# rafaelvp-db/databricks-distributed-deep-learning

Measured on AMD Instinct MI355X. Metric: ResNet-50 images/sec (whole node), higher is better.
Workload: dtype bf16

## Files before the change

### csrc/kernels/skinny_gemm.hip

```cpp
#include "ddl_lds.h"

#include <algorithm>
#include <cstdlib>

namespace {

constexpr int TM = 64, NT = 256, NW = NT / 64;
enum Epi { EPI_PLAIN = 0, EPI_RES = 1, EPI_BNB = 2, EPI_RESBNB = 3 };
template <int EPI>
constexpr bool is_bnb() { return EPI == EPI_BNB || EPI == EPI_RESBNB; }
template <int N>
constexpr int mask_stride() { return TM * N / 8 > 1024 ? TM * N / 8 : 1024; }

struct SkParams {
    const bf16_t* A;
    const bf16_t* B;
    bf16_t* C;
    long M;
    int tiles, chunk;
    float* colstats;
    const bf16_t* res;
    const bf16_t* aux;
    const uint8_t* mask;
    const float* mean;
    const float* istd;
    uint32_t c_bytes;
};

template <int N, int K, int EPI>
__global__ __launch_bounds__(NT) void skinny_gemm_k(SkParams p) {
    constexpr int NCF = N / 64;
    constexpr int KK = K / 32;
    constexpr int ABYTES = TM * K * 2, BBYTES = N * K * 2, CBYTES = TM * N * 2;
    constexpr int OFF_A = BBYTES, OFF_C = OFF_A + 2 * ABYTES;
    constexpr int NCIMG = EPI == EPI_PLAIN ? 1 : 2;
    constexpr int OFF_M = OFF_C + NCIMG * CBYTES;
    constexpr int MS = mask_stride<N>();
    constexpr int LDS = OFF_M + (is_bnb<EPI>() ? 2 * MS : 0);
    __shared__ __attribute__((aligned(16))) char smem[LDS];
    const int tid = threadIdx.x, lane = tid & 63, wv = __builtin_amdgcn_readfirstlane(tid >> 6);
    const int g = lane >> 4, r16 = lane & 15;
    const int cb = wv * 16 * NCF;
    const uint32_t lds0 = (uint32_t)(uintptr_t)smem;
    const __amdgpu_buffer_rsrc_t crs = rsrc(p.C, p.c_bytes);
    const bf16_t* eop = (EPI == EPI_RES || EPI == EPI_RESBNB) ? p.res : p.aux;

    const int t0 = blockIdx.x * p.chunk, t1 = min(p.tiles, t0 + p.chunk);
    auto prefetch = [&](int t, int buf) {
        dma_rows<NW, K, TM>(p.A, (long)t * TM, p.M, smem + OFF_A + buf * ABYTES, wv, lane);
        if constexpr (EPI != EPI_PLAIN) dma_rows<NW, N, TM>(eop, (long)t * TM, p.M, smem + OFF_C + buf * CBYTES, wv, lane);
        if constexpr (is_bnb<EPI>()) {
            const long byte0 = (long)t * TM * (N / 8), last = p.M * (N / 8) - 4;
#pragma unroll
            for (int k = 0; k < TM * N / 8 / 256; ++k) {
                const long b = min(byte0 + (long)(k * 64 + lane) * 4, last);
                const uint8_t* src = p.mask ? p.mask + b : (const uint8_t*)p.A;
                glds4(src, smem + OFF_M + buf * MS + k * 256);
            }
        }
    };
    uint2 xa[4][NCF], xb[4][NCF];
    auto prefetch_x = [&](int t, uint2 (&dst)[4][NCF]) {
#pragma unroll
        for (int i = 0; i < 4; ++i) {
            const long row = min((long)t * TM + 16 * i + r16, p.M - 1);
#pragma unroll
            for (int j = 0; j < NCF; ++j)
                dst[i][j] = *reinterpret_cast<const uint2*>(p.aux + row * N + cb + 16 * j + 4 * g);
        }
    };
    dma_rows<NW, K, N>(p.B, 0, N, smem, wv, lane);
    if (t0 < t1) {
        prefetch(t0, 0);
        if constexpr (EPI == EPI_RESBNB) prefetch_x(t0, xa);
    }

    uint32_t aoff[4][KK], boff[NCF][KK];
#pragma unroll
    for (int kk = 0; kk < KK; ++kk) {
#pragma unroll
        for (int i = 0; i < 4; ++i) {
            const int r = 16 * i + r16;
            aoff[i][kk] = r * (K * 2) + (((kk * 4 + g) ^ (r & swm<K>())) << 4);
        }
#pragma unroll
        for (int j = 0; j < NCF; ++j) {
            const int r = cb + 16 * j + r16;
            boff[j][kk] = lds0 + r * (K * 2) + (((kk * 4 + g) ^ (r & swm<K>())) << 4);
        }
    }
    auto coff = [&](int i, int j) -> uint32_t {
        const int row = 16 * i + r16, c = (cb + 16 * j) / 8 + (g >> 1);
        return row * (N * 2) + ((c ^ (row & swm<N>())) << 4) + (g & 1) * 8;
    };

    float st_s[NCF][4], st_q[NCF][4];
#pragma unroll
    for (int j = 0; j < NCF; ++j)
#pragma unroll
        for (int e = 0; e < 4; ++e) st_s[j][e] = st_q[j][e] = 0.f;
    float bmu[NCF][4] = {}, bis[NCF][4] = {};
    if constexpr (is_bnb<EPI>()) {
#pragma unroll
        for (int j = 0; j < NCF; ++j) {
            load4(p.mean + cb + 16 * j + 4 * g, bmu[j]);
            load4(p.istd + cb + 16 * j + 4 * g, bis[j]);
        }
    }

    auto tile = [&](const int t, uint2 (&xc)[4][NCF], uint2 (&xn)[4][NCF]) __attribute__((always_inline)) {
        const int buf = (t - t0) & 1;
        if constexpr (EPI == EPI_RESBNB) {
            __builtin_amdgcn_s_waitcnt(0xF70 | (2 * NCF));
        } else {
            if (t == t0) asm volatile("s_waitcnt vmcnt(0)" ::: "memory");
            else asm volatile("s_waitcnt vmcnt(%0)" ::"n"(2 * NCF) : "memory");
        }
        __builtin_amdgcn_s_barrier();
        if (t + 1 < t1) prefetch(t + 1, buf ^ 1);
        if constexpr (EPI == EPI_RESBNB) prefetch_x(t + 1, xn);

        const uint32_t abase = lds0 + OFF_A + buf * ABYTES;
        f32x4 acc[4][NCF];
#pragma unroll
        for (int i = 0; i < 4; ++i)
#pragma unroll
            for (int j = 0; j < NCF; ++j) acc[i][j] = (f32x4){0.f, 0.f, 0.f, 0.f};
#pragma unroll
        for (int kk = 0; kk < KK; ++kk) {
            bf16x8 af[4], bfr[NCF];
#pragma unroll
            for (int i = 0; i < 4; ++i) af[i] = ds_read16(abase + aoff[i][kk]);
#pragma unroll
            for (int j = 0; j < NCF; ++j) bfr[j] = ds_read16(boff[j][kk]);
            asm volatile("s_waitcnt lgkmcnt(0)" ::: "memory");
            __builtin_amdgcn_sched_barrier(0);
#pragma unroll
            for (int i = 0; i < 4; ++i)
#pragma unroll
                for (int j = 0; j < NCF; ++j)
                    acc[i][j] = __builtin_amdgcn_mfma_f32_16x16x32_bf16(bfr[j], af[i], acc[i][j], 0, 0, 0);
            __builtin_amdgcn_sched_barrier(0);
        }

        const long m0 = (long)t * TM;
        const uint32_t cimg = lds0 + OFF_C + (EPI == EPI_PLAIN ? 0 : buf * CBYTES);
        uint32_t mwords[4][2] = {{~0u, ~0u}, {~0u, ~0u}, {~0u, ~0u}, {~0u, ~0u}};
        if constexpr (is_bnb<EPI>()) {
            if (p.mask) {
#pragma unroll
                for (int i = 0; i < 4; ++i) {
                    const uint32_t a = lds0 + OFF_M + buf * MS + (16 * i + r16) * (N / 8) + (cb & ~31) / 8;
                    if constexpr (NCF > 2) {
                        const uint2 w2 = ds_read8(a);
                        mwords[i][0] = w2.x;
                        mwords[i][1] = w2.y;
                    } else {
                        mwords[i][0] = ds_read32(a);
                    }
                }
            }
        }
        uint2 ev[4][NCF];
        if constexpr (EPI != EPI_PLAIN) {
#pragma unroll
            for (int i = 0; i < 4; ++i)
#pragma unroll
                for (int j = 0; j < NCF; ++j) ev[i][j] = ds_read8(cimg + coff(i, j));
        }
        asm volatile("s_waitcnt lgkmcnt(0)" ::: "memory");
        __builtin_amdgcn_sched_barrier(0);
#pragma unroll
        for (int i = 0; i < 4; ++i) {
            const bool ok = m0 + 16 * i + r16 < p.M;
#pragma unroll
            for (int j = 0; j < NCF; ++j) {
                float v[4] = {acc[i][j][0], acc[i][j][1], acc[i][j][2], acc[i][j][3]};
                float xv[4] = {0.f, 0.f, 0.f, 0.f};
                if constexpr (EPI != EPI_PLAIN) {
                    xv[0] = __uint_as_float(ev[i][j].x << 16);
                    xv[1] = __uint_as_float(ev[i][j].x & 0xffff0000u);
                    xv[2] = __uint_as_float(ev[i][j].y << 16);
                    xv[3] = __uint_as_float(ev[i][j].y & 0xffff0000u);
                }
                if constexpr (EPI == EPI_RES || EPI == EPI_RESBNB) {
#pragma unroll
                    for (int e = 0; e < 4; ++e) v[e] += xv[e];
                }
                if constexpr (EPI == EPI_RESBNB) {
                    xv[0] = __uint_as_float(xc[i][j].x << 16);
                    xv[1] = __uint_as_float(xc[i][j].x & 0xffff0000u);
                    xv[2] = __uint_as_float(xc[i][j].y << 16);
                    xv[3] = __uint_as_float(xc[i][j].y & 0xffff0000u);
                }
                if constexpr (is_bnb<EPI>()) {
                    const uint32_t bits = mwords[i][(((cb & 31) + 16 * j) >> 5)] >> (((cb + 16 * j) & 16) + 4 * g);
#pragma unroll
                    for (int e = 0; e < 4; ++e) v[e] = ((bits >> e) & 1u) ? v[e] : 0.f;
                }
                const uint32_t lo = pack2bf(v[0], v[1]), hi = pack2bf(v[2], v[3]);
                ds_write8(cimg + coff(i, j), make_uint2(lo, hi));
                if (EPI != EPI_RES && ok) {
                    const float tq[4] = {__uint_as_float(lo << 16), __uint_as_float(lo & 0xffff0000u),
                                         __uint_as_float(hi << 16), __uint_as_float(hi & 0xffff0000u)};
#pragma unroll
                    for (int e = 0; e < 4; ++e) {
                        st_s[j][e] += tq[e];
                        st_q[j][e] += is_bnb<EPI>() ? tq[e] * xv[e] : tq[e] * tq[e];
                    }
                }
            }
        }
        asm volatile("s_waitcnt lgkmcnt(0)" ::: "memory");
        __builtin_amdgcn_s_barrier();
        constexpr int RPI = 1024 / (N * 2), CPR = N * 2 / 16;
#pragma unroll
        for (int qq = 0; qq < 2 * NCF; ++qq) {
            const int q = qq * 4 + wv;
            const int row = q * RPI + lane / CPR, c = lane % CPR;
            const u32x4 d = __builtin_bit_cast(u32x4, ds_read16(cimg + row * (N * 2) + ((c ^ (row & swm<N>())) << 4)));
            asm volatile("s_waitcnt lgkmcnt(0)" ::: "memory");
            __builtin_amdgcn_sched_barrier(0);
            const long grow = m0 + row;
            const uint32_t off = grow < p.M ? (uint32_t)((grow * N + c * 8) * 2) : 0x80000000u;
            __builtin_amdgcn_raw_buffer_store_b128(d, crs, (int)off, 0, 0);
        }
    };
    if constexpr (EPI == EPI_RESBNB) {
        __builtin_amdgcn_s_waitcnt(0xF70);
        for (int t = t0; t < t1; t += 2) {
            tile(t, xa, xb);
            if (t + 1 < t1) tile(t + 1, xb, xa);
        }
    } else {
        for (int t = t0; t < t1; ++t) tile(t, xa, xb);
    }

    if (EPI != EPI_RES && p.colstats) {
        asm volatile("s_waitcnt vmcnt(0)" ::: "memory");
        __syncthreads();
        float* red = reinterpret_cast<float*>(smem);
        for (int t = tid; t < 2 * N; t += NT) red[t] = 0.f;
        __syncthreads();
#pragma unroll
        for (int j = 0; j < NCF; ++j)
#pragma unroll
            for (int e = 0; e < 4; ++e) {
                float a = row16_sum(st_s[j][e]), b = row16_sum(st_q[j][e]);
                if constexpr (is_bnb<EPI>()) b = (b - bmu[j][e] * a) * bis[j][e];
                if (r16 == 0) {
                    const int col = cb + 16 * j + 4 * g + e;
                    atomicAdd(&red[col], a);
                    atomicAdd(&red[N + col], b);
                }
            }
        __syncthreads();
        for (int t = tid; t < 2 * N; t += NT) p.colstats[(long)blockIdx.x * 2 * N + t] = red[t];
    }
}

template <int N, int K, int EPI>
int launch(const SkParams& p0, int grid, hipStream_t st) {
    SkParams p = p0;
    constexpr int lds = N * K * 2 + 2 * TM * K * 2 + (EPI == EPI_PLAIN ? 1 : 2) * TM * N * 2 +
                        (is_bnb<EPI>() ? 2 * mask_stride<N>() : 0);
    const int per_cu = std::max(1, std::min(4, (160 * 1024) / lds));
    int g = grid > 0 ? grid : 256 * per_cu;
    g = std::min(g, p.tiles);
    p.chunk = (p.tiles + g - 1) / g;
    g = (p.tiles + p.chunk - 1) / p.chunk;
    hipLaunchKernelGGL((skinny_gemm_k<N, K, EPI>), dim3(g), dim3(NT), 0, st, p);
    return g;
}

}

DDL_API int ddl_skinny_gemm(const void* A, const void* B, void* C, long M, int N, int K, float* colstats,
                            const void* res, const void* aux, const uint8_t* mask, const float* mean,
                            const float* istd, int grid, hipStream_t stream) {
    if (M < 1 || M * (long)N * 2 >= (1l << 31)) return -1;
    const bool n256 = N == 256 && K == 64, n64 = N == 64 && K == 256;
    if (!n256 && !n64) return -1;
    if (res && !n256) return -1;
    if (aux && (!mean || !istd || (n256 && !res))) return -1;
    SkParams p{};
    p.A = (const bf16_t*)A;
    p.B = (const bf16_t*)B;
    p.C = (bf16_t*)C;
    p.M = M;
    p.tiles = (int)((M + TM - 1) / TM);
    p.colstats = colstats;
    p.res = (const bf16_t*)res;
    p.aux = (const bf16_t*)aux;
    p.mask = mask;
    p.mean = mean;
    p.istd = istd;
    p.c_bytes = (uint32_t)(M * N * 2);
    int g;
    if (n256) g = res ? (aux ? launch<256, 64, EPI_RESBNB>(p, grid, stream) : launch<256, 64, EPI_RES>(p, grid, stream))
                      : launch<256, 64, EPI_PLAIN>(p, grid, stream);
    else g = aux ? launch<64, 256, EPI_BNB>(p, grid, stream) : launch<64, 256, EPI_PLAIN>(p, grid, stream);
    const hipError_t e = hipGetLastError();
    if (e != hipSuccess) return -2 - (int)e;
    return (colstats && (!res || aux)) ? g : 0;
}
```

### databricks_distributed_deep_learning_amd/ops/_lib.py

```python
from __future__ import annotations

import ctypes
import os
from typing import Optional

import torch

_PKG_DIR = os.path.dirname(os.path.dirname(os.path.abspath(__file__)))
LIB_PATH = os.environ.get("DDL_NATIVE_LIB") or os.path.join(_PKG_DIR, "_native", "libddl_kernels.so")

_lib: Optional[ctypes.CDLL] = None
_load_error: Optional[str] = None
_mode = os.environ.get("DDL_NATIVE", "auto").lower()


class NativeUnavailable(RuntimeError):
    pass


def set_mode(mode: str) -> None:
    global _mode
    if mode not in ("auto", "on", "off"):
        raise ValueError(mode)
    _mode = mode
# ... 37 lines not shown

def load_error() -> Optional[str]:
    load()
    return _load_error


def use_native(*tensors: torch.Tensor) -> bool:
    if _mode == "off":
        return False
    if not all(t is None or t.is_cuda for t in tensors):
        return False
    if load() is None:
        raise NativeUnavailable(
            f"HIP kernel library unavailable on a GPU run: {_load_error}. "
            "Build it with `python csrc/build.py` or set DDL_NATIVE=off for stock PyTorch ops.")
    return True


def get() -> ctypes.CDLL:
    lib = load()
    if lib is None:
        raise NativeUnavailable(_load_error)
    return lib


def stream() -> ctypes.c_void_p:
    return ctypes.c_void_p(torch.cuda.current_stream().cuda_stream)


def ptr(t: Optional[torch.Tensor]) -> ctypes.c_void_p:
    return ctypes.c_void_p(0 if t is None else t.data_ptr())


def check(rc: int, what: str) -> None:
    if rc != 0:
        raise RuntimeError(f"native kernel {what} failed with HIP error {rc}")


P, I, L, F, U64 = ctypes.c_void_p, ctypes.c_int, ctypes.c_long, ctypes.c_float, ctypes.c_uint64
_SIGS = {
    "ddl_bn_stats_nblk": [L, I],
    "ddl_bn_bwd_nblk": [L, I],
    "ddl_bn_rows_sum": [P, I, I, P, P, P],
    "ddl_rows_sum_sink": [I, P, I, I, I, P, I, P, P],
    "ddl_bn_stats_partials": [I, P, L, I, P, P],
    "ddl_bn_bwd_partials": [I, P, P, P, P, P, L, I, I, P, P],
    "ddl_bn_bwd_finish": [I, P, P, P, P, P, P, L, L, I, I, P, P, P, P, P, P, P, I, P],
    "ddl_bn_bwd_from_partials": [I, P, I, P, L, P, P, P, P, P, L, I, P, P, P, P, P, I, P],
    "ddl_bn_partials_ws": [I, I],
    "ddl_bn_fwd_train": [I, P, L, I, P, P, P, P, F, F, P, P, P, P, P, P],
    "ddl_bn_eval_coeffs": [I, I, P, P, P, P, F, P, P, P],
    "ddl_bn_apply": [I, P, P, P, P, P, L, I, I, P, P],
    "ddl_bn_apply2": [I, P, P, P, P, P, P, P, L, I, I, P, P],
    "ddl_bn_relu_maxpool": [I, P, P, P, P, P, P, I, I, I, I, I, I, P],
    "ddl_bn_bwd_pool_nblk": [],
    "ddl_bn_bwd_pool": [I, P, P, P, P, P, P, P, I, I, I, I, I, I, P, P, P, P, P, I, P],
    "ddl_bn_bwd_coef_from_partials": [I, P, I, P, L, P, P, L, I, P, P, P, I, P],
    "ddl_bn_bwd_apply_coef": [I, P, P, P, P, P, L, I, P, P],
    "ddl_bn_fwd_from_partials": [I, P, I, L, I, P, P, P, P, F, F, P, P, P, P, P, L],
    "ddl_conv_w_dgrad": [P, P, I, I, I, I, I, I, P, P, P],
    "ddl_conv_w_dgrad_batch": [P, P, I, P],
    "ddl_gelu_bwd_colsum": [I, P, P, P, L, I, P, P, I, I, P],
    "ddl_acc_f32": [I, P, P, L, P],
    "ddl_tanh_bwd": [I, P, P, P, L, P],
    "ddl_copy2d": [I, P, L, L, L, P, L, L, L, P],
    "ddl_add_into": [I, P, P, L, P],
    "ddl_zero": [P, L, P],
    "ddl_rows_add_row": [I, P, P, P, L, L, P],
    "ddl_seq_prepend_add": [I, P, P, P, P, L, L, L, P],
    "ddl_sort_ids_ok": [L, L],
    "ddl_sort_ids": [P, L, P, P, P],
    "ddl_drain_acc": [I, P, P, L, P],
    "ddl_acc_grad": [I, P, P, L, I, I, P],
    "ddl_softmax_topk": [I, P, L, I, I, P, P, P, P],
    "ddl_gemm_conv_multi": [I, I, P, P, P, P, P, L, I, P, P],
    "ddl_conv3x3": [P, P, P, I, I, I, I, I, P, P, P, P, P, P, I, P],
    "ddl_conv3x3_wgrad": [P, P, P, I, I, I, I, I, P, L, I, I, I, P],
    "ddl_stem_wgrad": [P, P, P, I, I, I, I, I, I, I, P, L, I, I, I, P],
    "ddl_stem_fwd": [P, P, P, I, I, I, I, P, I, P],
    "ddl_s2d_input": [P, I, I, I, I, I, P, I, I, P],
    "ddl_s2d_weight": [P, I, I, I, I, P, I, I, P],
    "ddl_skinny_gemm": [P, P, P, L, I, I, P, P, P, P, P, P, I, P],
    "ddl_stream_gemm": [P, P, P, L, I, I, P, P, P, P, P, P, I, P],
    "ddl_stream_wgrad_ws": [I, I],
    "ddl_conv3_bwd_grid": [L, I],
    "ddl_conv3_bwd": [P, P, P, P, P, P, P, P, P, P, P, P, P, P, L, P, I, I, L, I, I, I, P],
    "ddl_bn_bwd": [I, P, P, P, P, P, P, L, I, I, P, P, P, P, P, P, I, P],
    "ddl_ln_supported": [I],
    "ddl_ln_fwd": [I, P, P, L, P, P, P, P, P, L, I, F, U64, F, P],
    "ddl_ln_bwd_nblk": [L],
    "ddl_ln_bwd": [I, P, P, P, L, P, P, P, P, P, P, P, L, I, I, P, U64, F, P, P, P, P],
    "ddl_gelu_fwd": [I, P, P, L, P],
    "ddl_gelu_bwd": [I, P, P, P, L, P],
    "ddl_dropout": [I, P, P, L, U64, F, P],
    "ddl_colsum_nblk": [L],
    "ddl_colsum": [I, P, L, I, P, P, I, I, P],
    "ddl_softmax_ce": [I, P, P, L, I, P, P, P, P],
    "ddl_scale_by": [I, P, P, P, L, P],
    "ddl_maxpool_fwd": [I, P, P, P, I, I, I, I, I, I, I, I, I, P],
    "ddl_maxpool_bwd": [I, P, P, P, I, I, I, I, I, I, I, I, I, P],
    "ddl_avgpool_fwd": [I, P, P, I, I, I, P],
    "ddl_avgpool_bwd": [I, P, P, I, I, I, P],
    "ddl_embedding_fwd": [I, P, P, P, L, I, P],
    "ddl_embedding_bwd": [I, P, P, P, P, L, L, I, I, P],
    "ddl_embedding_bwd_sorted": [I, P, P, P, P, P, L, I, I, P],
    "ddl_sgd_step": [I, P, P, I, P, P, P, I, P, F, F, F, I, I, P],
    "ddl_adamw_step": [I, P, P, I, P, P, P, P, I, P, F, F, F, F, F, F, F, F, F, P],
    "ddl_lamb_step": [I, P, P, I, P, P, P, P, I, P, F, F, F, F, F, F, F, F, F, P, P],
    "ddl_sumsq": [I, P, L, P, P],
    "ddl_lamb_phase1": [I, P, P, P, P, P, I, P, F, F, F, F, F, F, F, F, P, P],
    "ddl_lamb_phase2": [P, I, P, P, P, P, I, F, F, F, F, F, P, P],
}
_fns = {}


def fn(name: str):
    f = _fns.get(name)
    if f is None:
        f = getattr(get(), name)
        if name in _SIGS:
            f.argtypes = _SIGS[name]
        f.restype = ctypes.c_int
        _fns[name] = f
    return f


def call(name: str, *args) -> None:
    rc = fn(name)(*args, stream())
    if rc != 0:
        raise RuntimeError(f"native kernel {name} failed with code {rc}")


def register(sigs: dict) -> None:
    _SIGS.update(sigs)


def dcode(t: torch.Tensor) -> int:
    if t.dtype == torch.bfloat16:
        return 1
    if t.dtype == torch.float32:
        return 0
    raise TypeError(f"native kernels support fp32/bf16, got {t.dtype}")


def p(t: Optional[torch.Tensor]) -> int:
    return 0 if t is None else t.data_ptr()


def grad_sink(param) -> Optional[torch.Tensor]:
    if param is None:
        return None
    return getattr(param, "_ddl_main_grad", None)


def grad_ready(param) -> None:
    cb = getattr(param, "_ddl_grad_ready", None)
    if cb is not None:
        cb()


import contextlib as _contextlib

_WGRAD_STREAM = os.environ.get("DDL_WGRAD_STREAM", "0") != "0"
_side: dict = {}


# ... 38 lines not shown
```

### databricks_distributed_deep_learning_amd/ops/_native_conv.py

```python
from __future__ import annotations

import ctypes
import os

import torch
import torch.nn.functional as F

from . import _lib
from ._lib import grad_ready, grad_sink
from ._native_gemm import MODE_CONV, MODE_CONVW, MODE_NN, MODE_NT, MODE_TN, gemm, plan, stats_rows_max
from ._native_norm import _BN_BWD_EPI, _BN_BWD_EPI_RES


def _desc(N, H, W, C, P, Q, stride, h_off, w_off, h_step, w_step, R, S, OH, OW, ostep=1, oa=0, ob=0):
    return [N, H, W, C, P, Q, stride, h_off, w_off, h_step, w_step, R, S, OH, OW, ostep, oa, ob]


STATS_MIN_K = int(os.environ.get("DDL_BN_STATS_MIN_K", "0"))
_DGRAD_NT = os.environ.get("DDL_DGRAD_NT", "1") != "0"


_CONV3X3 = os.environ.get("DDL_CONV3X3", "1") != "0"


# ... 47 lines not shown
        return None
    if part is not None and part.numel() < 256 * 2 * N:
        return None
    args = (_lib.p(bnb.x), _lib.p(bnb.mask), _lib.p(bnb.mean), _lib.p(bnb.istd)) if bnb is not None else (0, 0, 0, 0)
    rc = _lib.fn("ddl_stream_gemm")(a.data_ptr(), b.data_ptr(), c.data_ptr(), M, N, K, _lib.p(part), _lib.p(res),
                                    *args, 0, _lib.stream())
    if rc == -1:
        return None
    if rc < 0:
        raise RuntimeError(f"ddl_stream_gemm failed: {rc}")
    return rc


def _skinny(a, b, c, part=None, res=None, bnb=None):
    if not a.is_cuda:
        return None
    M, K = a.shape
    N = b.shape[0]
    if (N, K) in _STREAM_SHAPES:
        return _stream(a, b, c, part, res, bnb)
    if (N, K) not in ((256, 64), (64, 256)) or tuple(c.shape) != (M, N) or b.shape[1] != K:
        return None
    ts = [a, b, c] + ([res] if res is not None else []) + ([bnb.x] if bnb is not None else [])
    if any(t.dtype != torch.bfloat16 or not t.is_contiguous() for t in ts):
        return None
    if (res is not None and N != 256) or (bnb is not None and N != 64 and res is None):
        return None
    if res is not None and tuple(res.shape) != (M, N) or bnb is not None and bnb.x.numel() != M * N:
        return None
    if part is not None and part.numel() < 1024 * 2 * N:
        return None
    args = (_lib.p(bnb.x), _lib.p(bnb.mask), _lib.p(bnb.mean), _lib.p(bnb.istd)) if bnb is not None else (0, 0, 0, 0)
    rc = _lib.fn("ddl_skinny_gemm")(a.data_ptr(), b.data_ptr(), c.data_ptr(), M, N, K, _lib.p(part), _lib.p(res),
                                    *args, 0, _lib.stream())
    if rc == -1:
        return None
    if rc < 0:
        raise RuntimeError(f"ddl_skinny_gemm failed: {rc}")
    return rc


def _direct3x3_rows(M):
    return max(stats_rows_max(M), 256)


def _fwd(x, w, stride, pad, bias=None, act=None, residual=None, stats=None):
    N, H, W_, C = x.shape
    K, R, S, _ = w.shape
    if (bias is None and act is None and residual is None and x.is_cuda
            and _direct3x3_ok(x.shape, w.shape, stride, pad)):
        y = torch.empty(N, H, W_, K, dtype=x.dtype, device=x.device)
        use_stats = stats is not None
        part = torch.empty(_direct3x3_rows(N * H * W_) * 2 * K, dtype=torch.float32, device=x.device) \
            if use_stats else None
        r = _direct3x3(x, w, y, part)
        if part is not None:
            stats.set(y, part, r)
        return y
    P = (H + 2 * pad - R) // stride + 1
    Q = (W_ + 2 * pad - S) // stride + 1
    y = torch.empty(N, P, Q, K, dtype=x.dtype, device=x.device)
    M = N * P * Q
    part = None
    kernel = None
    plain11 = R == 1 and S == 1 and stride == 1 and pad == 0
    desc = None if plain11 else _desc(N, H, W_, C, P, Q, stride, -pad, -pad, 1, 1, R, S, P, Q)
    if stats is not None and bias is None and act is None and residual is None and x.is_cuda:
        if R * S * C >= STATS_MIN_K:
            use = True
        elif plain11:
            use = plan(MODE_NT, x, C, w, C, y, K, M, K, C) == "big"
        else:
            use = plan(MODE_CONV, x, 0, w, R * S * C, y, K, M, K, R * S * C, conv=desc) == "big"
        if use:
            part = torch.empty(stats_rows_max(M) * 2 * K, dtype=torch.float32, device=x.device)
            kernel = None if R * S * C >= STATS_MIN_K else "big"
    if plain11 and bias is None and act is None and residual is None and x.is_cuda:
        sk_part = torch.empty(max(stats_rows_max(M), 1024) * 2 * K, dtype=torch.float32, device=x.device) \
            if part is not None else None
        rows = _skinny(x.view(M, C), w.view(K, C), y.view(M, K), part=sk_part)
        if rows is not None:
            if part is not None:
                stats.set(y, sk_part, rows)
            return y
    if plain11:
        r = gemm(MODE_NT, x, C, w, C, y, K, M, K, C, bias=bias, act=act, residual=residual, colstats=part,
                 kernel=kernel)
    else:
        r = gemm(MODE_CONV, x, 0, w, R * S * C, y, K, M, K, R * S * C, bias=bias, act=act, residual=residual,
                 conv=desc, colstats=part, kernel=kernel)
    if part is not None:
        stats.set(y, part, r)
    return y


class _WDgradCache:

    def __init__(self):
        self.jobs = {}
        self.gen = None
        self.table = None

    def _build(self):
        rows, blk = [], 0
        for w, rs, ss, out, _ in self.jobs.values():
            K, R, S, C = w.shape
            gk, gc = (K + 31) // 32, (C + 31) // 32
            r8 = list(rs) + [0] * (8 - len(rs))
            s8 = list(ss) + [0] * (8 - len(ss))
            rows.append([w.data_ptr(), out.data_ptr(), K, R, S, C, len(rs), len(ss), gk, gc, blk] + r8 + s8)
            blk += gk * gc * len(rs) * len(ss)
        host = torch.tensor(rows, dtype=torch.int64)
        self.table = (host.to(next(iter(self.jobs.values()))[0].device), host, len(rows))

    def get(self, w, rs, ss, generation):
        key = (w.data_ptr(), tuple(w.shape), tuple(rs), tuple(ss))
        if generation != self.gen:
            self.gen = generation
            if self.jobs:
                if self.table is None:
                    self._build()
                dev, host, n = self.table
                rc = _lib.fn("ddl_conv_w_dgrad_batch")(dev.data_ptr(), host.data_ptr(), n, _lib.stream())
                if rc != 0:
                    raise RuntimeError(f"ddl_conv_w_dgrad_batch failed: {rc}")
                for job in self.jobs.values():
                    job[4] = (generation, job[0]._version)
        job = self.jobs.get(key)
        stamp = (generation, w._version)
        if job is not None and job[4] == stamp:
            return job[3]
        if job is None:
            job = [w, tuple(rs), tuple(ss), None, None]
            self.jobs[key] = job
            self.table = None
        job[3] = _w_dgrad_once(w, rs, ss, job[3])
        job[4] = stamp
        return job[3]


def _w_dgrad(w, rs, ss, param=None):
    ref = getattr(param, "_ddl_arena", None) if param is not None else None
    arena = ref() if ref is not None else None
    if arena is not None and param.data_ptr() == w.data_ptr() and w.is_cuda \
            and not torch.cuda.is_current_stream_capturing():
        cache = getattr(arena, "_ddl_wdg", None)
        if cache is None:
            cache = arena._ddl_wdg = _WDgradCache()
        return cache.get(w, rs, ss, arena.generation)
    return _w_dgrad_once(w, rs, ss)


def _w_dgrad_once(w, rs, ss, out=None):
    K, R, S, C = w.shape
    if out is None:
        out = torch.empty(C, len(rs), len(ss), K, dtype=w.dtype, device=w.device)
    ra = (ctypes.c_int * len(rs))(*rs)
    sa = (ctypes.c_int * len(ss))(*ss)
    rc = _lib.fn("ddl_conv_w_dgrad")(w.data_ptr(), out.data_ptr(), K, R, S, C, len(rs), len(ss), ra, sa,
                                     _lib.stream())
    if rc != 0:
        raise RuntimeError(f"ddl_conv_w_dgrad failed: {rc}")
    return out


def _bnb_dgrad(mode, dy, lda, wt, ldb, dx, M, C, K, conv, residual, hint):
# ... 488 lines not shown
```

### databricks_distributed_deep_learning_amd/ops/_native_norm.py

```python
from __future__ import annotations

import os
from types import SimpleNamespace
from typing import Optional

import torch

from . import _lib
from ._native_elementwise import new_seed
from ._lib import call, dcode, grad_ready, grad_sink, p

_BN_BWD_EPI = os.environ.get("DDL_BN_BWD_EPI", "1") != "0"
_BN_BWD_EPI_RES = os.environ.get("DDL_BN_BWD_EPI", "1") not in ("0", "nores")


def _bn_supported(C: int) -> bool:
    return C % 8 == 0 and 256 % (C // 8) == 0


def _group_sum(row: torch.Tensor, group) -> None:
    import torch.distributed as dist
    from ..parallel import comm as _comm
    eng = _comm.active()
    if eng is not None and row.is_cuda and (group is None or group is dist.group.WORLD
                                            or dist.get_world_size(group) == eng.world):
        eng.wait_upto(eng.all_reduce(row))
        return
    dist.all_reduce(row, op=dist.ReduceOp.SUM, group=group)


def _bn_train_stats(x, weight, bias, running_mean, running_var, momentum, eps, given, stats) -> None:
    C = x.shape[-1]
    M = x.numel() // C
    dt = dcode(x)
    f32 = dict(dtype=torch.float32, device=x.device)
    if given is not None:
        part, nblk = given
        ws = torch.empty(-(-nblk // 32) * 2 * C, **f32) if nblk > 32 else None
        call("ddl_bn_fwd_from_partials", dt, p(part), nblk, M, C, p(weight), p(bias), p(running_mean),
             p(running_var), float(momentum), float(eps), p(stats[0]), p(stats[1]), p(stats[2]), p(stats[3]),
             p(ws), 0 if ws is None else ws.numel())
    else:
        nblk = _lib.fn("ddl_bn_stats_nblk")(M, C)
        part = torch.empty(nblk * 2 * C, **f32)
        call("ddl_bn_fwd_train", dt, p(x), M, C, p(weight), p(bias), p(running_mean), p(running_var),
             float(momentum), float(eps), p(part), p(stats[0]), p(stats[1]), p(stats[2]), p(stats[3]))


class _BatchNormTrain(torch.autograd.Function):
    @staticmethod
    def forward(ctx, x, weight, bias, running_mean, running_var, momentum, eps, relu, residual, bridge=None,
                pre=None, group=None):
        ctx.bridge = bridge
        ctx.group = group
        ctx.c3 = _conv3_hint(x) if group is None else None
        x = x.contiguous()
        C = x.shape[-1]
        M = x.numel() // C
        dt = dcode(x)
        f32 = dict(dtype=torch.float32, device=x.device)
        stats = torch.empty(4, C, **f32)
        given = pre.take_for(x) if pre is not None else None
        if group is not None:
            import torch.distributed as dist
            world = dist.get_world_size(group)
            if given is not None:
                part, nblk = given
                ws = torch.empty(-(-nblk // 32) * 2 * C, **f32)
            else:
                nblk = _lib.fn("ddl_bn_stats_nblk")(M, C)
                part = torch.empty((nblk + -(-nblk // 32)) * 2 * C, **f32)
                call("ddl_bn_stats_partials", dt, p(x), M, C, p(part))
                ws = None
            row = torch.empty(2 * C, **f32)
            call("ddl_bn_rows_sum", p(part), nblk, 2 * C, p(row), p(ws))
            _group_sum(row, group)
            call("ddl_bn_fwd_from_partials", dt, p(row), 1, M * world, C, p(weight), p(bias), p(running_mean),
                 p(running_var), float(momentum), float(eps), p(stats[0]), p(stats[1]), p(stats[2]), p(stats[3]),
                 None, 0)
            ctx.m_total = M * world
        else:
            _bn_train_stats(x, weight, bias, running_mean, running_var, momentum, eps, given, stats)
        res = residual.contiguous() if residual is not None else None
        y = torch.empty_like(x)
        mask = torch.empty(x.numel() // 8, dtype=torch.uint8, device=x.device) if relu else None
        call("ddl_bn_apply", dt, p(x), p(res), p(stats[2]), p(stats[3]), p(y), x.numel(), C, int(relu), p(mask))
        ctx.relu = bool(relu)
        ctx.has_res = residual is not None
        ctx.params = (weight, bias)
        ctx.save_for_backward(x, mask, weight, stats)
        ctx.bnb = None
        if _BN_BWD_EPI and x.dtype == torch.bfloat16:
            from .bridge import BNBackward
            ctx.bnb = BNBackward(x, mask, stats[0], stats[1])
            y._ddl_bnb = ctx.bnb
        return y

    @staticmethod
    def backward(ctx, dy):
        x, mask, weight, stats = ctx.saved_tensors
        dx, dgamma, dbeta, dres = _bn_backward(ctx, dy, x, mask, weight, stats)
        return dx, dgamma, dbeta, None, None, None, None, None, dres, None, None, None


def _conv3_hint(x):
    hint = getattr(x, "_ddl_c3", None)
    if hint is None or not x.is_contiguous() or x.dtype != torch.bfloat16 or not x.requires_grad:
        return None
    return hint


def _bn_backward(ctx, dy, x, mask, weight, stats):
    dy = dy.contiguous()
    C = x.shape[-1]
    M = x.numel() // C
    nblk = _lib.fn("ddl_bn_bwd_nblk")(M, C)
    f32 = dict(dtype=torch.float32, device=x.device)
    part = torch.empty((nblk + -(-nblk // 32)) * 2 * C, **f32)
    coef = torch.empty(3 * C, **f32)
    sg, sb = grad_sink(ctx.params[0]), grad_sink(ctx.params[1])
    direct = sg is not None and sb is not None
    if direct:
        dgamma, dbeta = sg, sb
    else:
        dgamma = torch.empty_like(weight) if weight is not None else None
        dbeta = torch.empty_like(weight) if weight is not None else None
    given = ctx.bnb.take_for(dy) if ctx.bnb is not None else None
    ctx.bnb = None
    c3 = getattr(ctx, "c3", None)
    fold = c3 is not None and given is not None and ctx.group is None and weight is not None
    dx = None if fold else torch.empty_like(x)
    dres = torch.empty_like(x) if ctx.has_res and (given is None or ctx.group is not None) else None
    if given is not None:
        gpart, nrows = given
        if ctx.group is not None:
            row = torch.empty(2 * C, **f32)
            call("ddl_bn_rows_sum", p(gpart), nrows, 2 * C, p(row), None)
            local = row.clone()
            _group_sum(row, ctx.group)
            call("ddl_bn_bwd_finish", dcode(x), p(dy), None, p(x), p(stats[0]), p(stats[1]), p(weight), M,
                 ctx.m_total, C, 0, p(row), p(local), p(dgamma), p(dbeta), p(coef), p(dx), p(dres), int(direct))
        elif fold:
            ws = gpart[nrows * 2 * C:]
            call("ddl_bn_bwd_coef_from_partials", dcode(x), p(gpart), nrows, p(ws), ws.numel(), p(stats[1]),
                 p(weight), M, C, p(dgamma), p(dbeta), p(coef), int(direct))
            c3.park(dy, x, stats[0], stats[1], coef)
            dx = dy
            if ctx.has_res:
                dres = dy
        else:
            ws = gpart[nrows * 2 * C:]
            call("ddl_bn_bwd_from_partials", dcode(x), p(gpart), nrows, p(ws), ws.numel(), p(dy), p(x),
                 p(stats[0]), p(stats[1]), p(weight), M, C, p(dgamma), p(dbeta), p(coef), p(dx), None,
                 int(direct))
            if ctx.has_res:
                dres = dy
    elif ctx.group is not None:
        call("ddl_bn_bwd_partials", dcode(x), p(dy), p(mask), p(x), p(stats[0]), p(stats[1]), M, C,
             int(ctx.relu), p(part))
        row = torch.empty(2 * C, **f32)
        call("ddl_bn_rows_sum", p(part), nblk, 2 * C, p(row), None)
        local = row.clone()
        _group_sum(row, ctx.group)
        call("ddl_bn_bwd_finish", dcode(x), p(dy), p(mask), p(x), p(stats[0]), p(stats[1]), p(weight), M,
             ctx.m_total, C, int(ctx.relu), p(row), p(local), p(dgamma), p(dbeta), p(coef), p(dx), p(dres),
             int(direct))
    else:
        call("ddl_bn_bwd", dcode(x), p(dy), p(mask), p(x), p(stats[0]), p(stats[1]), p(weight), M, C,
             int(ctx.relu), p(part), p(dgamma), p(dbeta), p(coef), p(dx), p(dres), int(direct))
    if direct:
        grad_ready(ctx.params[0])
        grad_ready(ctx.params[1])
        dgamma = dbeta = None
    if dres is not None and ctx.bridge is not None:
        ctx.bridge.put(dres)
        dres = None
    return dx, dgamma, dbeta, dres


class _BatchNormAddBNTrain(torch.autograd.Function):

    @staticmethod
    def forward(ctx, x, weight, bias, running_mean, running_var, momentum, eps, x2, weight2, bias2, running_mean2,
                running_var2, momentum2, eps2, pre=None, pre2=None):
        ctx.c3 = _conv3_hint(x)
        x, x2 = x.contiguous(), x2.contiguous()
        C = x.shape[-1]
        f32 = dict(dtype=torch.float32, device=x.device)
        stats = torch.empty(4, C, **f32)
        stats2 = torch.empty(4, C, **f32)
        _bn_train_stats(x, weight, bias, running_mean, running_var, momentum, eps,
                        pre.take_for(x) if pre is not None else None, stats)
        _bn_train_stats(x2, weight2, bias2, running_mean2, running_var2, momentum2, eps2,
                        pre2.take_for(x2) if pre2 is not None else None, stats2)
        y = torch.empty_like(x)
        mask = torch.empty(x.numel() // 8, dtype=torch.uint8, device=x.device)
        call("ddl_bn_apply2", dcode(x), p(x), p(x2), p(stats[2]), p(stats[3]), p(stats2[2]), p(stats2[3]), p(y),
             x.numel(), C, 1, p(mask))
        ctx.bridge, ctx.group, ctx.relu, ctx.has_res = None, None, True, True
        ctx.params, ctx.params2 = (weight, bias), (weight2, bias2)
        ctx.save_for_backward(x, mask, weight, stats, x2, weight2, stats2)
        ctx.bnb = None
        if _BN_BWD_EPI and x.dtype == torch.bfloat16:
            from .bridge import BNBackward
            ctx.bnb = BNBackward(x, mask, stats[0], stats[1])
            y._ddl_bnb = ctx.bnb
        return y

    @staticmethod
    def backward(ctx, dy):
        x, mask, weight, stats, x2, weight2, stats2 = ctx.saved_tensors
        dx, dgamma, dbeta, dres = _bn_backward(ctx, dy, x, mask, weight, stats)
        c2 = SimpleNamespace(bnb=None, group=None, has_res=False, relu=False, params=ctx.params2, bridge=None)
        dx2, dgamma2, dbeta2, _ = _bn_backward(c2, dres, x2, None, weight2, stats2)
        return (dx, dgamma, dbeta, None, None, None, None, dx2, dgamma2, dbeta2, None, None, None, None, None, None)


class _BNReluMaxPoolTrain(torch.autograd.Function):

    @staticmethod
    def forward(ctx, x, weight, bias, running_mean, running_var, momentum, eps, pre=None):
        x = x.contiguous()
        N, H, W, C = x.shape
        P, Q = H // 2, W // 2
        stats = torch.empty(4, C, dtype=torch.float32, device=x.device)
        _bn_train_stats(x, weight, bias, running_mean, running_var, momentum, eps,
                        pre.take_for(x) if pre is not None else None, stats)
        y = torch.empty(N, P, Q, C, dtype=x.dtype, device=x.device)
        idx = torch.empty(N, P, Q, C, dtype=torch.uint8, device=x.device)
        mask = torch.empty(x.numel() // 8, dtype=torch.uint8, device=x.device)
        call("ddl_bn_relu_maxpool", dcode(x), p(x), p(stats[2]), p(stats[3]), p(y), p(idx), p(mask), N, H, W, C, P, Q)
        ctx.params = (weight, bias)
        ctx.save_for_backward(x, mask, weight, stats, idx)
        return y

    @staticmethod
    def backward(ctx, dy):
        x, mask, weight, stats, idx = ctx.saved_tensors
        N, H, W, C = x.shape
        dy = dy.contiguous()
        if not _FUSED_STEM_BWD:
            da = torch.empty_like(x)
            call("ddl_maxpool_bwd", dcode(dy), p(dy), p(idx), p(da), N, H, W, C, H // 2, W // 2, 3, 2, 1)
            c = SimpleNamespace(bnb=None, group=None, has_res=False, relu=True, params=ctx.params, bridge=None)
            dx, dgamma, dbeta, _ = _bn_backward(c, da, x, mask, weight, stats)
            return dx, dgamma, dbeta, None, None, None, None, None
        nblk = _lib.fn("ddl_bn_bwd_pool_nblk")()
        f32 = dict(dtype=torch.float32, device=x.device)
        part = torch.empty((nblk + -(-nblk // 32)) * 2 * C, **f32)
        coef = torch.empty(3 * C, **f32)
        dx = torch.empty_like(x)
        sg, sb = grad_sink(ctx.params[0]), grad_sink(ctx.params[1])
        direct = sg is not None and sb is not None
        dgamma, dbeta = (sg, sb) if direct else (torch.empty_like(weight), torch.empty_like(weight))
        call("ddl_bn_bwd_pool", dcode(x), p(dy), p(idx), p(mask), p(x), p(stats[0]), p(stats[1]), p(weight), N, H, W,
             C, H // 2, W // 2, p(part), p(dgamma), p(dbeta), p(coef), p(dx), int(direct))
        if direct:
            grad_ready(ctx.params[0])
            grad_ready(ctx.params[1])
            dgamma = dbeta = None
        return dx, dgamma, dbeta, None, None, None, None, None


def bn_relu_maxpool(x, weight, bias, running_mean, running_var, momentum, eps, pre=None):
    N, H, W, C = x.shape
    if (not _bn_supported(C) or x.dtype not in (torch.bfloat16, torch.float32)
            or H % 2 or W % 2 or weight is None):
        return None
    if weight.dtype != x.dtype:
        weight, bias = weight.to(x.dtype), bias.to(x.dtype)
    return _BNReluMaxPoolTrain.apply(x, weight, bias, running_mean, running_var, momentum, eps, pre)


_FUSED_STEM_BWD = os.environ.get("DDL_FUSED_STEM_BWD", "0") != "0"


def batch_norm_add_bn(x, weight, bias, running_mean, running_var, momentum, eps, x2, weight2, bias2,
                      running_mean2, running_var2, momentum2, eps2, pre=None, pre2=None):
    C = x.shape[-1]
    if (not _bn_supported(C) or x.dtype not in (torch.bfloat16, torch.float32) or x2.dtype != x.dtype
            or x2.shape != x.shape or weight is None or weight2 is None):
# ... 153 lines not shown
```

### databricks_distributed_deep_learning_amd/ops/bridge.py

```python
from __future__ import annotations

import os
from typing import Optional

import torch

CONV3_FUSED = os.environ.get("DDL_CONV3_BWD_FUSED", "1") != "0"
CONV3_SHAPES = ((256, 64),)


class GradBridge:
    __slots__ = ("grad", "closed")

    def __init__(self):
        self.grad: Optional[torch.Tensor] = None
        self.closed = False

    def put(self, g: torch.Tensor) -> None:
        if self.grad is not None:
            raise RuntimeError("GradBridge: gradient already pending (bridge reused within one backward?)")
        self.grad = g

    def offer(self, g: torch.Tensor) -> bool:
        if self.closed:
            return False
        self.put(g)
        return True

    def take(self) -> Optional[torch.Tensor]:
        g, self.grad = self.grad, None
        self.closed = True
        return g


class _BridgeJoin(torch.autograd.Function):

    @staticmethod
    def forward(ctx, x, bridge):
        ctx.bridge = bridge
        return x.view_as(x)

    @staticmethod
    def backward(ctx, g):
        r = ctx.bridge.take()
        return (g if r is None else g + r.view_as(g)), None


def join(x: torch.Tensor, bridge: Optional[GradBridge]) -> torch.Tensor:
    return x if bridge is None else _BridgeJoin.apply(x, bridge)


class BNStats:
    __slots__ = ("ptr", "numel", "part", "nblk")

    def __init__(self):
        self.ptr = None
        self.numel = 0
        self.part = None
        self.nblk = 0

    def set(self, y: torch.Tensor, part: torch.Tensor, nblk: int) -> None:
        self.ptr, self.numel, self.part, self.nblk = y.data_ptr(), y.numel(), part, nblk

    def take_for(self, x: torch.Tensor):
        if self.part is None or self.ptr != x.data_ptr() or self.numel != x.numel():
            return None
        part, nblk = self.part, self.nblk
        self.part = None
        return part, nblk


class BNBackward:
    __slots__ = ("x", "mask", "mean", "istd", "dz", "part", "nrows")

    def __init__(self, x: torch.Tensor, mask: Optional[torch.Tensor], mean: torch.Tensor, istd: torch.Tensor):
        self.x, self.mask, self.mean, self.istd = x, mask, mean, istd
        self.dz = None
        self.part = None
        self.nrows = 0

    def set(self, dz: torch.Tensor, part: torch.Tensor, nrows: int) -> None:
        self.dz, self.part, self.nrows = dz, part, nrows

    def take_for(self, g: torch.Tensor):
        dz, part, nrows = self.dz, self.part, self.nrows
        self.dz = self.part = None
        if dz is None or dz.data_ptr() != g.data_ptr() or dz.numel() != g.numel():
            return None
        return part, nrows


class Conv3Fold:
    __slots__ = ("parked",)

    def __init__(self):
        self.parked = None

    def park(self, dz: torch.Tensor, x: torch.Tensor, mean: torch.Tensor, istd: torch.Tensor,
             coef: torch.Tensor) -> None:
        if self.parked is not None:
            raise RuntimeError("Conv3Fold: a gradient is already parked (hint reused within one backward?)")
        self.parked = (dz, x, mean, istd, coef)

    def take(self):
        parked, self.parked = self.parked, None
        return parked

    @staticmethod
    def is_parked(parked, g: torch.Tensor) -> bool:
        dz = parked[0]
        return dz.data_ptr() == g.data_ptr() and dz.numel() == g.numel() and dz.dtype == g.dtype
```

Measured before the change: 13020.

## Recompute conv3 1x1 GEMM fused with BN apply, residual, ReLU and mask

For 256x64 conv3 shapes, the forward BN-apply no longer reads the conv output. It recomputes the skinny GEMM from its inputs and fuses scale/shift, residual add (or second BN), ReLU and packed ReLU-mask writing into the GEMM epilogue. This trades a read of the large conv output tensor for extra matmul FLOPs on small K=64 inputs. It adds new epilogue variants, union params, and version checks so recompute only happens when the operands are unchanged.

```diff
diff --git a/csrc/kernels/skinny_gemm.hip b/csrc/kernels/skinny_gemm.hip
--- a/csrc/kernels/skinny_gemm.hip
+++ b/csrc/kernels/skinny_gemm.hip
@@ -6,11 +6,17 @@
 namespace {
 
 constexpr int TM = 64, NT = 256, NW = NT / 64;
-enum Epi { EPI_PLAIN = 0, EPI_RES = 1, EPI_BNB = 2, EPI_RESBNB = 3 };
+enum Epi { EPI_PLAIN = 0, EPI_RES = 1, EPI_BNB = 2, EPI_RESBNB = 3, EPI_BNRES = 4, EPI_BN2RES = 5 };
 template <int EPI>
 constexpr bool is_bnb() { return EPI == EPI_BNB || EPI == EPI_RESBNB; }
+template <int EPI>
+constexpr bool is_bnres() { return EPI == EPI_BNRES || EPI == EPI_BN2RES; }
+template <int EPI>
+constexpr bool has_stats() { return EPI != EPI_RES && !is_bnres<EPI>(); }
 template <int N>
 constexpr int mask_stride() { return TM * N / 8 > 1024 ? TM * N / 8 : 1024; }
+template <int N, int EPI>
+constexpr int tail_bytes() { return is_bnb<EPI>() ? 2 * mask_stride<N>() : is_bnres<EPI>() ? TM * N / 8 : 0; }
 
 struct SkParams {
     const bf16_t* A;
@@ -18,14 +24,38 @@
     bf16_t* C;
     long M;
     int tiles, chunk;
-    float* colstats;
+    union {
+        float* colstats;
+        const float* shift2;
+    };
     const bf16_t* res;
-    const bf16_t* aux;
-    const uint8_t* mask;
-    const float* mean;
-    const float* istd;
+    union {
+        const bf16_t* aux;
+        const float* scale2;
+    };
+    union {
+        const uint8_t* mask;
+        uint8_t* omask;
+    };
+    union {
+        const float* mean;
+        const float* scale;
+    };
+    union {
+        const float* istd;
+        const float* shift;
+    };
     uint32_t c_bytes;
 };
+
+__device__ __forceinline__ float mul_rounded(float a, float b) {
+    float m = a * b;
+    asm volatile("" : "+v"(m));
+    return m;
+}
+__device__ __forceinline__ void ds_write1(uint32_t addr, uint32_t v) {
+    asm volatile("ds_write_b8 %0, %1" ::"v"(addr), "v"(v) : "memory");
+}
 
 template <int N, int K, int EPI>
 __global__ __launch_bounds__(NT) void skinny_gemm_k(SkParams p) {
@@ -36,14 +66,15 @@
     constexpr int NCIMG = EPI == EPI_PLAIN ? 1 : 2;
     constexpr int OFF_M = OFF_C + NCIMG * CBYTES;
     constexpr int MS = mask_stride<N>();
-    constexpr int LDS = OFF_M + (is_bnb<EPI>() ? 2 * MS : 0);
+    constexpr int LDS = OFF_M + tail_bytes<N, EPI>();
+    constexpr int NST = 2 * NCF + (is_bnres<EPI>() ? 1 : 0);
     __shared__ __attribute__((aligned(16))) char smem[LDS];
     const int tid = threadIdx.x, lane = tid & 63, wv = __builtin_amdgcn_readfirstlane(tid >> 6);
     const int g = lane >> 4, r16 = lane & 15;
     const int cb = wv * 16 * NCF;
     const uint32_t lds0 = (uint32_t)(uintptr_t)smem;
     const __amdgpu_buffer_rsrc_t crs = rsrc(p.C, p.c_bytes);
-    const bf16_t* eop = (EPI == EPI_RES || EPI == EPI_RESBNB) ? p.res : p.aux;
+    const bf16_t* eop = (EPI == EPI_RES || EPI == EPI_RESBNB || is_bnres<EPI>()) ? p.res : p.aux;
 
     const int t0 = blockIdx.x * p.chunk, t1 = min(p.tiles, t0 + p.chunk);
     auto prefetch = [&](int t, int buf) {
@@ -107,6 +138,22 @@
             load4(p.istd + cb + 16 * j + 4 * g, bis[j]);
         }
     }
+    float bsc[NCF][4] = {}, bsh[NCF][4] = {}, bsc2[NCF][4] = {};
+    if constexpr (is_bnres<EPI>()) {
+#pragma unroll
+        for (int j = 0; j < NCF; ++j) {
+            load4(p.scale + cb + 16 * j + 4 * g, bsc[j]);
+            load4(p.shift + cb + 16 * j + 4 * g, bsh[j]);
+            if constexpr (EPI == EPI_BN2RES) {
+                float s2[4];
+                load4(p.scale2 + cb + 16 * j + 4 * g, bsc2[j]);
+                load4(p.shift2 + cb + 16 * j + 4 * g, s2);
+#pragma unroll
+                for (int e = 0; e < 4; ++e) bsh[j][e] += s2[e];
+            }
+        }
+    }
+    [[maybe_unused]] const __amdgpu_buffer_rsrc_t mrs = rsrc(p.omask, is_bnres<EPI>() ? p.c_bytes / 16 : 0);
 
     auto tile = [&](const int t, uint2 (&xc)[4][NCF], uint2 (&xn)[4][NCF]) __attribute__((always_inline)) {
         const int buf = (t - t0) & 1;
@@ -114,7 +161,7 @@
             __builtin_amdgcn_s_waitcnt(0xF70 | (2 * NCF));
         } else {
             if (t == t0) asm volatile("s_waitcnt vmcnt(0)" ::: "memory");
-            else asm volatile("s_waitcnt vmcnt(%0)" ::"n"(2 * NCF) : "memory");
+            else asm volatile("s_waitcnt vmcnt(%0)" ::"n"(NST) : "memory");
         }
         __builtin_amdgcn_s_barrier();
         if (t + 1 < t1) prefetch(t + 1, buf ^ 1);
@@ -187,6 +234,23 @@
 #pragma unroll
                     for (int e = 0; e < 4; ++e) v[e] += xv[e];
                 }
+                if constexpr (is_bnres<EPI>()) {
+                    const uint32_t xl = pack2bf(v[0], v[1]), xh = pack2bf(v[2], v[3]);
+                    const float x3[4] = {__uint_as_float(xl << 16), __uint_as_float(xl & 0xffff0000u),
+                                         __uint_as_float(xh << 16), __uint_as_float(xh & 0xffff0000u)};
+#pragma unroll
+                    for (int e = 0; e < 4; ++e) {
+                        float t;
+                        if constexpr (EPI == EPI_BN2RES) {
+                            t = mul_rounded(x3[e], bsc[j][e]) + mul_rounded(xv[e], bsc2[j][e]);
+                            t = t + bsh[j][e];
+                        } else {
+                            t = __builtin_fmaf(x3[e], bsc[j][e], bsh[j][e]);
+                            t = t + xv[e];
+                        }
+                        v[e] = fmaxf(t, 0.f);
+                    }
+                }
                 if constexpr (EPI == EPI_RESBNB) {
                     xv[0] = __uint_as_float(xc[i][j].x << 16);
                     xv[1] = __uint_as_float(xc[i][j].x & 0xffff0000u);
@@ -200,7 +264,7 @@
                 }
                 const uint32_t lo = pack2bf(v[0], v[1]), hi = pack2bf(v[2], v[3]);
                 ds_write8(cimg + coff(i, j), make_uint2(lo, hi));
-                if (EPI != EPI_RES && ok) {
+                if (has_stats<EPI>() && ok) {
                     const float tq[4] = {__uint_as_float(lo << 16), __uint_as_float(lo & 0xffff0000u),
                                          __uint_as_float(hi << 16), __uint_as_float(hi & 0xffff0000u)};
 #pragma unroll
@@ -216,7 +280,7 @@
         constexpr int RPI = 1024 / (N * 2), CPR = N * 2 / 16;
 #pragma unroll
         for (int qq = 0; qq < 2 * NCF; ++qq) {
-            const int q = qq * 4 + wv;
+            const int q = is_bnres<EPI>() ? wv * (2 * NCF) + qq : qq * 4 + wv;
             const int row = q * RPI + lane / CPR, c = lane % CPR;
             const u32x4 d = __builtin_bit_cast(u32x4, ds_read16(cimg + row * (N * 2) + ((c ^ (row & swm<N>())) << 4)));
             asm volatile("s_waitcnt lgkmcnt(0)" ::: "memory");
@@ -224,6 +288,24 @@
             const long grow = m0 + row;
             const uint32_t off = grow < p.M ? (uint32_t)((grow * N + c * 8) * 2) : 0x80000000u;
             __builtin_amdgcn_raw_buffer_store_b128(d, crs, (int)off, 0, 0);
+            if constexpr (is_bnres<EPI>()) {
+                uint32_t bits = 0;
+#pragma unroll
+                for (int e = 0; e < 8; ++e) {
+                    const uint32_t h = e & 1 ? d[e >> 1] & 0xffff0000u : d[e >> 1] << 16;
+                    bits |= (__uint_as_float(h) > 0.f ? 1u : 0u) << e;
+                }
+                ds_write1(lds0 + OFF_M + wv * (TM / NW * N / 8) + qq * 64 + lane, bits);
+            }
+        }
+        if constexpr (is_bnres<EPI>()) {
+            static_assert(N == 256, "8 mask bytes per lane cover the wave's 16 rows");
+            const uint2 mb = ds_read8(lds0 + OFF_M + wv * (TM / NW * N / 8) + lane * 8);
+            asm volatile("s_waitcnt lgkmcnt(0)" ::: "memory");
+            __builtin_amdgcn_sched_barrier(0);
+            const long grow = m0 + 16 * wv + lane / 4;
+            const uint32_t off = grow < p.M ? (uint32_t)(grow * (N / 8) + (lane & 3) * 8) : 0x80000000u;
+            __builtin_amdgcn_raw_buffer_store_b64((u32x2){mb.x, mb.y}, mrs, (int)off, 0, 0);
         }
     };
     if constexpr (EPI == EPI_RESBNB) {
@@ -236,7 +318,7 @@
         for (int t = t0; t < t1; ++t) tile(t, xa, xb);
     }
 
-    if (EPI != EPI_RES && p.colstats) {
+    if (has_stats<EPI>() && p.colstats) {
         asm volatile("s_waitcnt vmcnt(0)" ::: "memory");
         __syncthreads();
         float* red = reinterpret_cast<float*>(smem);
@@ -262,8 +344,7 @@
 template <int N, int K, int EPI>
 int launch(const SkParams& p0, int grid, hipStream_t st) {
     SkParams p = p0;
-    constexpr int lds = N * K * 2 + 2 * TM * K * 2 + (EPI == EPI_PLAIN ? 1 : 2) * TM * N * 2 +
-                        (is_bnb<EPI>() ? 2 * mask_stride<N>() : 0);
+    constexpr int lds = N * K * 2 + 2 * TM * K * 2 + (EPI == EPI_PLAIN ? 1 : 2) * TM * N * 2 + tail_bytes<N, EPI>();
     const int per_cu = std::max(1, std::min(4, (160 * 1024) / lds));
     int g = grid > 0 ? grid : 256 * per_cu;
     g = std::min(g, p.tiles);
@@ -304,3 +385,27 @@
     if (e != hipSuccess) return -2 - (int)e;
     return (colstats && (!res || aux)) ? g : 0;
 }
+
+DDL_API int ddl_skinny_gemm_bnres(const void* A, const void* B, const void* res, const float* scale,
+                                  const float* shift, const float* scale2, const float* shift2, void* Y,
+                                  uint8_t* mask, long M, int N, int K, int grid, hipStream_t stream) {
+    if (M < 1 || M * (long)N * 2 >= (1l << 31)) return -1;
+    if (N != 256 || K != 64 || !res || !scale || !shift || !mask || (scale2 != nullptr) != (shift2 != nullptr)) return -1;
+    SkParams p{};
+    p.A = (const bf16_t*)A;
+    p.B = (const bf16_t*)B;
+    p.C = (bf16_t*)Y;
+    p.M = M;
+    p.tiles = (int)((M + TM - 1) / TM);
+    p.res = (const bf16_t*)res;
+    p.c_bytes = (uint32_t)(M * N * 2);
+    p.scale = scale;
+    p.shift = shift;
+    p.scale2 = scale2;
+    p.shift2 = shift2;
+    p.omask = mask;
+    if (scale2) launch<256, 64, EPI_BN2RES>(p, grid, stream);
+    else launch<256, 64, EPI_BNRES>(p, grid, stream);
+    const hipError_t e = hipGetLastError();
+    return e != hipSuccess ? -2 - (int)e : 0;
+}
diff --git a/databricks_distributed_deep_learning_amd/ops/_lib.py b/databricks_distributed_deep_learning_amd/ops/_lib.py
--- a/databricks_distributed_deep_learning_amd/ops/_lib.py
+++ b/databricks_distributed_deep_learning_amd/ops/_lib.py
@@ -143,6 +143,7 @@
     "ddl_s2d_weight": [P, I, I, I, I, P, I, I, P],
     "ddl_skinny_gemm": [P, P, P, L, I, I, P, P, P, P, P, P, I, P],
     "ddl_stream_gemm": [P, P, P, L, I, I, P, P, P, P, P, P, I, P],
+    "ddl_skinny_gemm_bnres": [P, P, P, P, P, P, P, P, P, L, I, I, I, P],
     "ddl_stream_wgrad_ws": [I, I],
     "ddl_conv3_bwd_grid": [L, I],
     "ddl_conv3_bwd": [P, P, P, P, P, P, P, P, P, P, P, P, P, P, L, P, I, I, L, I, I, I, P],
diff --git a/databricks_distributed_deep_learning_amd/ops/_native_conv.py b/databricks_distributed_deep_learning_amd/ops/_native_conv.py
--- a/databricks_distributed_deep_learning_amd/ops/_native_conv.py
+++ b/databricks_distributed_deep_learning_amd/ops/_native_conv.py
@@ -153,6 +153,9 @@
         if rows is not None:
             if part is not None:
                 stats.set(y, sk_part, rows)
+            from . import bridge as B
+            if B.CONV3_FWD_RECOMPUTE and (K, C) in B.CONV3_RECOMPUTE_SHAPES:
+                y._ddl_c3r = B.Conv3Recompute(y, x, w)
             return y
     if plain11:
         r = gemm(MODE_NT, x, C, w, C, y, K, M, K, C, bias=bias, act=act, residual=residual, colstats=part,
diff --git a/databricks_distributed_deep_learning_amd/ops/_native_norm.py b/databricks_distributed_deep_learning_amd/ops/_native_norm.py
--- a/databricks_distributed_deep_learning_amd/ops/_native_norm.py
+++ b/databricks_distributed_deep_learning_amd/ops/_native_norm.py
@@ -54,6 +54,7 @@
         ctx.bridge = bridge
         ctx.group = group
         ctx.c3 = _conv3_hint(x) if group is None else None
+        c3r = getattr(x, "_ddl_c3r", None) if group is None and relu and residual is not None else None
         x = x.contiguous()
         C = x.shape[-1]
         M = x.numel() // C
@@ -84,7 +85,8 @@
         res = residual.contiguous() if residual is not None else None
         y = torch.empty_like(x)
         mask = torch.empty(x.numel() // 8, dtype=torch.uint8, device=x.device) if relu else None
-        call("ddl_bn_apply", dt, p(x), p(res), p(stats[2]), p(stats[3]), p(y), x.numel(), C, int(relu), p(mask))
+        if not _apply_recompute(c3r, x, res, stats, None, y, mask):
+            call("ddl_bn_apply", dt, p(x), p(res), p(stats[2]), p(stats[3]), p(y), x.numel(), C, int(relu), p(mask))
         ctx.relu = bool(relu)
         ctx.has_res = residual is not None
         ctx.params = (weight, bias)
@@ -101,6 +103,26 @@
         x, mask, weight, stats = ctx.saved_tensors
         dx, dgamma, dbeta, dres = _bn_backward(ctx, dy, x, mask, weight, stats)
         return dx, dgamma, dbeta, None, None, None, None, None, dres, None, None, None
+
+
+def _apply_recompute(hint, x, res, stats, stats2, y, mask) -> bool:
+    ops = hint.operands_for(x) if hint is not None else None
+    if (ops is None or x.dtype != torch.bfloat16 or res is None or res.dtype != x.dtype
+            or res.shape != x.shape or not res.is_contiguous()):
+        return False
+    a, w = ops
+    N, K = w.shape[0], a.shape[-1]
+    M = x.numel() // N
+    if x.shape[-1] != N or a.numel() != M * K or w.numel() != N * K:
+        return False
+    s2 = (p(stats2[2]), p(stats2[3])) if stats2 is not None else (0, 0)
+    rc = _lib.fn("ddl_skinny_gemm_bnres")(p(a), p(w), p(res), p(stats[2]), p(stats[3]), *s2, p(y), p(mask), M, N, K,
+                                          0, _lib.stream())
+    if rc == -1:
+        return False
+    if rc < 0:
+        raise RuntimeError(f"ddl_skinny_gemm_bnres failed: {rc}")
+    return True
 
 
 def _conv3_hint(x):
@@ -184,6 +206,7 @@
     def forward(ctx, x, weight, bias, running_mean, running_var, momentum, eps, x2, weight2, bias2, running_mean2,
                 running_var2, momentum2, eps2, pre=None, pre2=None):
         ctx.c3 = _conv3_hint(x)
+        c3r = getattr(x, "_ddl_c3r", None)
         x, x2 = x.contiguous(), x2.contiguous()
         C = x.shape[-1]
         f32 = dict(dtype=torch.float32, device=x.device)
@@ -195,8 +218,9 @@
                         pre2.take_for(x2) if pre2 is not None else None, stats2)
         y = torch.empty_like(x)
         mask = torch.empty(x.numel() // 8, dtype=torch.uint8, device=x.device)
-        call("ddl_bn_apply2", dcode(x), p(x), p(x2), p(stats[2]), p(stats[3]), p(stats2[2]), p(stats2[3]), p(y),
-             x.numel(), C, 1, p(mask))
+        if not _apply_recompute(c3r, x, x2, stats, stats2, y, mask):
+            call("ddl_bn_apply2", dcode(x), p(x), p(x2), p(stats[2]), p(stats[3]), p(stats2[2]), p(stats2[3]), p(y),
+                 x.numel(), C, 1, p(mask))
         ctx.bridge, ctx.group, ctx.relu, ctx.has_res = None, None, True, True
         ctx.params, ctx.params2 = (weight, bias), (weight2, bias2)
         ctx.save_for_backward(x, mask, weight, stats, x2, weight2, stats2)
diff --git a/databricks_distributed_deep_learning_amd/ops/bridge.py b/databricks_distributed_deep_learning_amd/ops/bridge.py
--- a/databricks_distributed_deep_learning_amd/ops/bridge.py
+++ b/databricks_distributed_deep_learning_amd/ops/bridge.py
@@ -7,6 +7,8 @@
 
 CONV3_FUSED = os.environ.get("DDL_CONV3_BWD_FUSED", "1") != "0"
 CONV3_SHAPES = ((256, 64),)
+CONV3_FWD_RECOMPUTE = os.environ.get("DDL_CONV3_FWD_RECOMPUTE", "1") != "0"
+CONV3_RECOMPUTE_SHAPES = ((256, 64),)
 
 
 class GradBridge:
@@ -90,6 +92,20 @@
         return part, nrows
 
 
+class Conv3Recompute:
+    __slots__ = ("ptr", "numel", "a", "w", "versions")
+
+    def __init__(self, y: torch.Tensor, a: torch.Tensor, w: torch.Tensor):
+        self.ptr, self.numel, self.a, self.w = y.data_ptr(), y.numel(), a, w
+        self.versions = (y._version, a._version, w._version)
+
+    def operands_for(self, x: torch.Tensor):
+        if (self.ptr != x.data_ptr() or self.numel != x.numel()
+                or self.versions != (x._version, self.a._version, self.w._version)):
+            return None
+        return self.a, self.w
+
+
 class Conv3Fold:
     __slots__ = ("parked",)
 
```

Result: no change. 13130 (median of 6 runs) (+0.8%).
